# OxfordML/GPz

Hardware: AMD Instinct MI355X
Metric: objective+gradient evals/sec (higher is better)
Workload: dtype f64

## Files before the change

### gpz_amd/csrc/k_phi_quad.hip

```cpp
#include <float.h>
#include "gpz_dev.h"
#include "gpz_kernels.h"

template <int D>
struct PhiQuadShape {
    static constexpr int NT = D * (D + 1) / 2;
    static constexpr int NF = 1 + D + NT;
    static constexpr int NK = (NF + 3) / 4;
    static constexpr int CS = 4 * NK;
};

int phi_quad_stride(int de) { return 4 * ((1 + de + de * (de + 1) / 2 + 3) / 4); }
bool phi_quad_fits(int kind, int de, int mp, int k) { return kind == GPZ_KIND_COV && (de == 8 || de == 10) && mp > 256 && k == 1; }

template <int D>
__global__ __launch_bounds__(64) void k_phi_quad_coef(const double *__restrict__ Rc, const double *__restrict__ P,
                                                        const double *__restrict__ xmu, const double *__restrict__ fmx, int m, int mp,
                                                        double *__restrict__ Cq, double *__restrict__ blockmax,
                                                        unsigned *__restrict__ ticket, double *__restrict__ bound,
                                                        int *__restrict__ route) {
    constexpr int NT = PhiQuadShape<D>::NT, NF = PhiQuadShape<D>::NF, CS = PhiQuadShape<D>::CS, NP = NT + D;
    const int j = blockIdx.x * 64 + threadIdx.x;
    double bj = 0.0;
    if (j < m) {
        double R[NT], pq[D], u[D], uh[D];
        const double *rj = Rc + (size_t)j * NP;
#pragma unroll
        for (int e = 0; e < NT; ++e) R[e] = rj[e];
#pragma unroll
        for (int a = 0; a < D; ++a) pq[a] = P[(size_t)j * D + a] - xmu[a];
#pragma unroll
        for (int a = 0; a < D; ++a) {
            double s = 0.0, sh = 0.0;
#pragma unroll
            for (int b = a; b < D; ++b) {
                const double r = R[a * D - a * (a - 1) / 2 + (b - a)];
                s = fma(r, pq[b], s);
                sh = fma(fabs(r), fabs(pq[b]), sh);
            }
            u[a] = s; uh[a] = sh;
        }
        double *o = Cq + (size_t)j * CS;
        double c0 = 0.0, c0h = 0.0;
#pragma unroll
        for (int a = 0; a < D; ++a) { c0 = fma(u[a], u[a], c0); c0h = fma(uh[a], uh[a], c0h); }
        o[0] = -0.5 * c0;
        double bs = fmx[0] * (0.5 * c0h);
#pragma unroll
        for (int a = 0; a < D; ++a) {
            double s = 0.0, sh = 0.0;
#pragma unroll
            for (int r = 0; r <= a; ++r) {
                const double v = R[r * D - r * (r - 1) / 2 + (a - r)];
                s = fma(v, u[r], s);
                sh = fma(fabs(v), uh[r], sh);
            }
            o[1 + a] = s;
            bs = fma(fmx[1 + a], sh, bs);
        }
#pragma unroll
        for (int a = 0; a < D; ++a)
#pragma unroll
            for (int b = a; b < D; ++b) {
                double s = 0.0, sh = 0.0;
#pragma unroll
                for (int r = 0; r <= a; ++r) {
                    const double va = R[r * D - r * (r - 1) / 2 + (a - r)], vb = R[r * D - r * (r - 1) / 2 + (b - r)];
                    s = fma(va, vb, s);
                    sh = fma(fabs(va), fabs(vb), sh);
                }
                const int f = 1 + D + a * D - a * (a - 1) / 2 + (b - a);
                const double sc = (a == b) ? 0.5 : 1.0;
                o[f] = -sc * s;
                bs = fma(fmx[f], sc * sh, bs);
            }
#pragma unroll
        for (int f = NF; f < CS; ++f) o[f] = 0.0;
        bj = (double)(NF + 2 * D + 6) * 0x1p-53 * bs;
        if (!(bj <= DBL_MAX)) bj = __longlong_as_double(0x7ff0000000000000LL);
    } else if (j < mp) {
        double *o = Cq + (size_t)j * CS;
#pragma unroll
        for (int f = 0; f < CS; ++f) o[f] = 0.0;
    }
#pragma unroll
    for (int off = 32; off > 0; off >>= 1) bj = fmax(bj, __shfl_xor(bj, off, 64));
    int last = 0;
    if (threadIdx.x == 0) {
        blockmax[blockIdx.x] = bj;
        __threadfence();
        last = atomicAdd(ticket, 1u) == gridDim.x - 1 ? 1 : 0;
        if (last) {
            __threadfence();
            double mx = 0.0;
            for (unsigned g = 0; g < gridDim.x; ++g) mx = fmax(mx, __hip_atomic_load(blockmax + g, __ATOMIC_RELAXED, __HIP_MEMORY_SCOPE_AGENT));
            *bound = mx;
            *route = mx <= GPZ_PHI_QUAD_TAU ? GPZ_PHI_ROUTE_QUAD : GPZ_PHI_ROUTE_EXACT;
            *ticket = 0u;
        }
    }
}

int launch_phi_quad_coef(hipStream_t st, const double *Rc, const double *P, const double *xmu, const double *fmx, int m, int mp, int de,
                         double *Cq, double *blockmax, unsigned *ticket, double *bound, int *route) {
    dim3 g((mp + 63) / 64), b(64);
    switch (de) {
        case 8: hipLaunchKernelGGL(k_phi_quad_coef<8>, g, b, 0, st, Rc, P, xmu, fmx, m, mp, Cq, blockmax, ticket, bound, route); break;
        case 10: hipLaunchKernelGGL(k_phi_quad_coef<10>, g, b, 0, st, Rc, P, xmu, fmx, m, mp, Cq, blockmax, ticket, bound, route); break;
        default: return -1;
    }
    return 0;
}

struct PhiQuadKArgs {
    const double *Xs;
    const double *Cq;
    const int *route;
    int n, m, mp;
    const double *v, *bvec, *omega, *Y;
    double *Phi, *lnbeta, *wbeta;
    int jgroup;
    double *part;
    long ldp;
};

#ifndef GPZ_PHI_QUAD_RB
#define GPZ_PHI_QUAD_RB 2
#endif
#ifndef GPZ_PHI_QUAD_WGS
#define GPZ_PHI_QUAD_WGS 3
#endif

template <int D, int RB>
__global__ __launch_bounds__(256, GPZ_PHI_QUAD_WGS) void k_phi_quad(PhiQuadKArgs a) {
    constexpr int NF = PhiQuadShape<D>::NF, NK = PhiQuadShape<D>::NK, CS = PhiQuadShape<D>::CS, XL = D + 2;
    constexpr int NPB = 16 * CS;
    constexpr int NLD = (NPB + 255) / 256;
    if (*a.route != GPZ_PHI_ROUTE_QUAD) return;
    __shared__ double cq[2][NPB];
    __shared__ unsigned char pia[CS], pib[CS];
    const int tid = threadIdx.x, lane = tid & 63, wave = tid >> 6, li = lane & 15, lk = lane >> 4;
    const long row0 = ((long)blockIdx.x * 4 + wave) * (16 * RB);

    if (tid < CS) {
        const int f = tid;
        int ia = 0, ib = 0;
        if (f >= NF) ia = ib = XL - 1;
        else if (f >= 1) {
            if (f <= D) ia = f;
            else {
                int e2 = f - 1 - D, aa = 0;
                while (e2 >= D - aa) { e2 -= D - aa; ++aa; }
                ia = aa + 1; ib = aa + e2 + 1;
            }
        }
        pia[f] = (unsigned char)ia; pib[f] = (unsigned char)ib;
    }
    const int jlo = blockIdx.y * a.jgroup;
    const int jhi = min(a.mp, jlo + a.jgroup);
    double stg[NLD];
    auto pload = [&](int j0) {
#pragma unroll
        for (int q = 0; q < NLD; ++q) {
            const int e = tid + 256 * q;
            stg[q] = e < NPB ? a.Cq[(size_t)j0 * CS + e] : 0.0;
        }
    };
    auto pstore = [&](int buf) {
#pragma unroll
        for (int q = 0; q < NLD; ++q) {
            const int e = tid + 256 * q;
            if (e < NPB) cq[buf][e] = stg[q];
        }
    };
    pload(jlo);
    pstore(0);
    __syncthreads();

    double F[RB][NK];
#pragma unroll
    for (int ks = 0; ks < NK; ++ks) {
        const int ia = pia[4 * ks + lk], ib = pib[4 * ks + lk];
#pragma unroll
        for (int rb = 0; rb < RB; ++rb) {
            const long i = row0 + 16 * rb + li;
            const double *xr = a.Xs + (size_t)i * XL;
            F[rb][ks] = xr[ia] * xr[ib];
        }
    }
    double sv[RB][4];
#pragma unroll
    for (int rb = 0; rb < RB; ++rb)
#pragma unroll
        for (int r = 0; r < 4; ++r) sv[rb][r] = 0.0;

    int cur = 0;
    for (int j0 = jlo; j0 < jhi; j0 += 16, cur ^= 1) {
        const bool more = j0 + 16 < jhi;
        if (more) pload(j0 + 16);
        const int j = j0 + li;
        const double vj = (a.v && j < a.m) ? a.v[j] : 0.0;
        d4_t acc[RB];
#pragma unroll
        for (int rb = 0; rb < RB; ++rb) acc[rb] = d4_t{0.0, 0.0, 0.0, 0.0};
        const double *cb = &cq[cur][li * CS + lk];
#pragma unroll
        for (int ks = 0; ks < NK; ++ks) {
            const double b = cb[4 * ks];
#pragma unroll
            for (int rb = 0; rb < RB; ++rb) acc[rb] = MFMA_F64(F[rb][ks], b, acc[rb]);
        }
        double ph[RB][4];
#pragma unroll
        for (int rb = 0; rb < RB; ++rb) {
#pragma unroll
            for (int r = 0; r < 4; ++r) {
                const long i = row0 + 16 * rb + lk + 4 * r;
                const double e = exp(fmin(acc[rb][r], 0.0));
                ph[rb][r] = i < a.n ? e : 0.0;
                sv[rb][r] = fma(ph[rb][r], vj, sv[rb][r]);
            }
        }
        if (j0 + 16 > a.m) {
#pragma unroll
            for (int rb = 0; rb < RB; ++rb) {
#pragma unroll
                for (int r = 0; r < 4; ++r) {
                    const double y = a.Y ? a.Y[row0 + 16 * rb + lk + 4 * r] : 0.0;
                    if (j >= a.m) ph[rb][r] = j == a.m ? y : 0.0;
                }
            }
        }
        double *const po = a.Phi + (size_t)(row0 + lk) * a.mp + j;
#pragma unroll
        for (int rb = 0; rb < RB; ++rb) {
#pragma unroll
            for (int r = 0; r < 4; ++r) po[(size_t)(16 * rb + 4 * r) * a.mp] = ph[rb][r];
        }
        if (more) pstore(cur ^ 1);
        __syncthreads();
    }

#pragma unroll
    for (int rb = 0; rb < RB; ++rb)
#pragma unroll
        for (int r = 0; r < 4; ++r) {
#pragma unroll
            for (int off = 1; off < 16; off <<= 1) sv[rb][r] += __shfl_xor(sv[rb][r], off, 64);
        }
    if (li != 0) return;
#pragma unroll
    for (int rb = 0; rb < RB; ++rb)
#pragma unroll
        for (int r = 0; r < 4; ++r) {
            const long i = row0 + 16 * rb + lk + 4 * r;
            if (a.part) {
                if (i < a.ldp) {
                    a.part[((size_t)blockIdx.y * 2 + 0) * a.ldp + i] = sv[rb][r];
                    a.part[((size_t)blockIdx.y * 2 + 1) * a.ldp + i] = 0.0;
                }
                continue;
            }
            const bool valid = i < a.n;
            const double lb = a.bvec[0] + sv[rb][r];
            a.lnbeta[i] = valid ? lb : 0.0;
            if (a.wbeta) {
                const double om = a.omega ? a.omega[i] : 1.0;
                a.wbeta[i] = valid ? om * exp(-lb) : 0.0;
            }
        }
}

template <int D>
static int launch_phi_quad_d(hipStream_t st, const PhiArgs &a, const double *Xs, const double *Cq) {
    constexpr int RB = GPZ_PHI_QUAD_RB, JB = 16;
    const int rows_per_wg = 4 * 16 * RB;
    if (a.n_pad <= 0 || a.n_pad % rows_per_wg != 0 || a.n_pad > a.ldx) return -1;
    const int nwg = a.n_pad / rows_per_wg;
    int ngroup = 1;
    if (a.part && nwg < 1024) {
        int maxg = a.mp / (4 * JB);
        if (maxg > a.part_groups) maxg = a.part_groups;
        ngroup = phi_pick_groups(nwg, a.mp, JB, 2, 16, maxg < 1 ? 1 : maxg);
    }
    int jgroup = ((a.mp + ngroup - 1) / ngroup + JB - 1) / JB * JB;
    ngroup = (a.mp + jgroup - 1) / jgroup;
    PhiQuadKArgs q{};
    q.Xs = Xs; q.Cq = Cq; q.route = a.route; q.n = a.n; q.m = a.m; q.mp = a.mp;
    q.v = a.v; q.bvec = a.b; q.omega = a.omega; q.Y = a.Y;
    q.Phi = a.Phi; q.lnbeta = a.lnbeta; q.wbeta = a.wbeta;
    q.jgroup = jgroup; q.part = ngroup > 1 ? a.part : nullptr; q.ldp = (long)a.n_pad;
    hipLaunchKernelGGL((k_phi_quad<D, RB>), dim3(nwg, ngroup), dim3(256), 0, st, q);
    if (q.part)
        launch_phi_finalize(st, q.part, ngroup, a, a.route, GPZ_PHI_ROUTE_QUAD);
    return hipGetLastError() == hipSuccess ? 0 : -1;
}

int launch_phi_quad(hipStream_t st, const PhiArgs &a, const double *Xs, const double *Cq) {
    if (a.k != 1 || a.mp % 16 != 0 || !a.route || a.wgtab || !a.Phi || !a.lnbeta || a.w || a.phiw) return -1;
    switch (a.d) {
        case 8: return launch_phi_quad_d<8>(st, a, Xs, Cq);
        case 10: return launch_phi_quad_d<10>(st, a, Xs, Cq);
        default: return -1;
    }
}
```

### gpz_amd/csrc/k_gemm.hip

```cpp
#include <type_traits>
#include "gpz_dev.h"
#include "gpz_kernels.h"

#ifdef GPZ_GEMM_TRACE
__device__ unsigned long long *g_gemm_trace = nullptr;
#define GPZ_TRACE_MARK(slot)                                                                                              \
    do {                                                                                                                  \
        if (g_gemm_trace && (threadIdx.x & 63) == 0)                                                                      \
            g_gemm_trace[((size_t)item * 8 + (threadIdx.x >> 6)) * 6 + (slot)] = __builtin_amdgcn_s_memtime();       \
    } while (0)
#else
#define GPZ_TRACE_MARK(slot) do { } while (0)
#endif
typedef float f4_t __attribute__((ext_vector_type(4)));
typedef float f2_t __attribute__((ext_vector_type(2)));
#ifndef GPZ_F32_FLUSH
#define GPZ_F32_FLUSH 8
#endif
template <typename OT> struct MfmaOf;
template <> struct MfmaOf<double> {
    typedef d4_t acc_t;
    typedef d2_t pair_t;
    static __device__ __forceinline__ acc_t run(double a, double b, acc_t c) { return MFMA_F64(a, b, c); }
};
template <> struct MfmaOf<float> {
    typedef f4_t acc_t;
    typedef f2_t pair_t;
    static __device__ __forceinline__ acc_t run(float a, float b, acc_t c) { return __builtin_amdgcn_mfma_f32_16x16x4f32(a, b, c, 0, 0, 0); }
};
template <typename OT>
__device__ __forceinline__ typename MfmaOf<OT>::pair_t to_pair(const f2_t v) {
    typename MfmaOf<OT>::pair_t r;
    r.x = (OT)v.x;
    r.y = (OT)v.y;
    return r;
}
template <typename BT> struct Pair2 { typedef d2_t t; };
template <> struct Pair2<float> { typedef f2_t t; };
template <typename OT>
__device__ __forceinline__ typename MfmaOf<OT>::pair_t to_pair(const d2_t v) {
    typename MfmaOf<OT>::pair_t r;
    r.x = (OT)v.x;
    r.y = (OT)v.y;
    return r;
}

template <bool WEIGHTED, int WC, bool DIAGT, typename OT>
__device__ __forceinline__ void syrk_body(const double *__restrict__ Phi, int ld, const double *__restrict__ wgt,
                                          int mp, int i0, int j0, int r_begin, int r_end,
                                          double *__restrict__ out, OT (*sA)[16][LDS_LD128],
                                          OT (*sB)[16][LDS_LD128], OT (*sW)[16]) {
    constexpr int NT = 128 * WC;
    constexpr int NI = 8 / WC;
    constexpr int Q = 1024 / NT;
    constexpr bool diag_tile = DIAGT;
    constexpr bool PRESCALE = WEIGHTED;
    const int tid = threadIdx.x, lane = tid & 63, wave = tid >> 6;
    const int wr = wave / WC, wc = wave % WC;

    constexpr bool F32 = std::is_same<OT, float>::value;
    typedef typename MfmaOf<OT>::acc_t acc_t;
    typedef typename MfmaOf<OT>::pair_t pair_t;
    acc_t acc[4][NI];
    d4_t acc64[F32 ? 4 : 1][F32 ? NI : 1];
#pragma unroll
    for (int a = 0; a < 4; ++a)
#pragma unroll
        for (int b = 0; b < NI; ++b) {
            acc[a][b] = (acc_t){0, 0, 0, 0};
            if (F32) acc64[a][b] = (d4_t){0.0, 0.0, 0.0, 0.0};
        }
    auto flush = [&]() {
        if constexpr (F32) {
#pragma unroll
            for (int a = 0; a < 4; ++a)
#pragma unroll
                for (int b = 0; b < NI; ++b) {
#pragma unroll
                    for (int r = 0; r < 4; ++r) acc64[a][b][r] += (double)acc[a][b][r];
                    acc[a][b] = (acc_t){0, 0, 0, 0};
                }
        }
    };

    d2_t ra[Q], rb[Q];
    double rw = 0.0, rwq[PRESCALE ? Q : 1];
    const int ca = min(i0 + (tid & 63) * 2, mp - 2), cb = min(j0 + (tid & 63) * 2, mp - 2);
    const unsigned voa = (unsigned)(((tid >> 6) * ld + ca) * 8), vob = (unsigned)(((tid >> 6) * ld + cb) * 8);
    const unsigned vow = (unsigned)((PRESCALE ? (tid >> 6) : (tid & 15)) * 8);
    const size_t qsp = (size_t)(NT / 64) * ld * 8, ksp = (size_t)16 * ld * 8;
    const char *pp = reinterpret_cast<const char *>(Phi + (size_t)r_begin * ld);
    const char *pw = reinterpret_cast<const char *>(WEIGHTED ? wgt + r_begin : nullptr);
    auto gload = [&]() {
        unsigned oa = voa, ob = vob, ow = vow;
        asm volatile("" : "+v"(oa), "+v"(ob), "+v"(ow));
#pragma unroll
        for (int q = 0; q < Q; ++q) {
            ra[q] = *reinterpret_cast<const d2_t *>(pp + q * qsp + oa);
            if (!diag_tile) rb[q] = *reinterpret_cast<const d2_t *>(pp + q * qsp + ob);
            if (PRESCALE) rwq[q] = *reinterpret_cast<const double *>(pw + q * (NT / 64) * 8 + ow);
        }
        if (WEIGHTED && !PRESCALE && tid < 16) rw = *reinterpret_cast<const double *>(pw + ow);
        pp += ksp;
        if (WEIGHTED) pw += 16 * 8;
    };
    auto lstore = [&](int buf) {
#pragma unroll
        for (int q = 0; q < Q; ++q) {
            int idx = q * NT + tid;
            int row = idx >> 6, c = (idx & 63) * 2;
            if (diag_tile) *reinterpret_cast<pair_t *>(&sB[buf][row][c]) = to_pair<OT>(ra[q]);
            else *reinterpret_cast<pair_t *>(&sB[buf][row][c]) = to_pair<OT>(rb[q]);
            if (PRESCALE) { ra[q].x *= rwq[q]; ra[q].y *= rwq[q]; }
            *reinterpret_cast<pair_t *>(&sA[buf][row][c]) = to_pair<OT>(ra[q]);
        }
        if (WEIGHTED && !PRESCALE && tid < 16) sW[buf][tid] = (OT)rw;
    };

    const int nstage = (r_end > r_begin) ? (r_end - r_begin) / 16 : 0;
    if (nstage > 0) {
        gload();
        lstore(0);
        if (nstage > 1) gload();
    }
    __syncthreads();
    static_assert(!DIAGT || NI == 2, "diagonal-tile wave roles are written for the 2 x 4 wave grid");
    constexpr int NA = 4, NB = DIAGT ? 5 : NI;
    int dra[5] = {0, 0, 0, 0, 0}, dcb[5] = {0, 0, 0, 0, 0};
    bool has5 = false;
    if (DIAGT) {
        const int wv = __builtin_amdgcn_readfirstlane(wave);
        const unsigned RA[8] = {0x00000u, 0x11111u, 0x22222u, 0x33333u, 0x77000u, 0x66611u, 0x55552u, 0x44444u};
        const unsigned CB[8] = {0x43210u, 0x54321u, 0x65432u, 0x76543u, 0x77765u, 0x77676u, 0x77657u, 0x77654u};
        has5 = wv < 4;
#pragma unroll
        for (int p = 0; p < 5; ++p) {
            dra[p] = (RA[wv] >> (4 * p)) & 15;
            dcb[p] = (CB[wv] >> (4 * p)) & 15;
        }
    }
    auto rdfrag = [&](int cur, int kk, OT (&a)[NA], OT (&b)[NB]) {
        const OT(*tA)[LDS_LD128] = sA[cur];
        const OT(*tB)[LDS_LD128] = sB[cur];
        const int krow = kk * 4 + (lane >> 4);
        if (DIAGT) {
#pragma unroll
            for (int p = 0; p < 4; ++p) a[p] = tA[krow][dra[p] * 16 + (lane & 15)];
#pragma unroll
            for (int p = 0; p < 5; ++p) b[p] = tB[krow][dcb[p] * 16 + (lane & 15)];
        } else {
#pragma unroll
            for (int mi = 0; mi < 4; ++mi) a[mi] = tA[krow][wr * 64 + mi * 16 + (lane & 15)];
#pragma unroll
            for (int ni = 0; ni < NI; ++ni) b[ni] = tB[krow][wc * (16 * NI) + ni * 16 + (lane & 15)];
        }
    };
    auto burst = [&](const OT (&a)[NA], const OT (&b)[NB]) {
        __builtin_amdgcn_s_setprio(1);
        if (DIAGT) {
#pragma unroll
            for (int p = 0; p < 4; ++p) acc[p][0] = MfmaOf<OT>::run(a[p], b[p], acc[p][0]);
            if (has5) acc[0][1] = MfmaOf<OT>::run(a[0], b[DIAGT ? 4 : 0], acc[0][1]);
        } else {
#pragma unroll
            for (int mi = 0; mi < 4; ++mi)
#pragma unroll
                for (int ni = 0; ni < NI; ++ni) acc[mi][ni] = MfmaOf<OT>::run(a[mi], b[ni], acc[mi][ni]);
        }
        __builtin_amdgcn_s_setprio(0);
    };
    OT fa0[NA] = {}, fb0[NB] = {}, fa1[NA] = {}, fb1[NB] = {};
    if (nstage > 0) rdfrag(0, 0, fa0, fb0);
    auto stage = [&](auto curc, int s) {
        constexpr int cur = decltype(curc)::value;
        rdfrag(cur, 1, fa1, fb1);
        __builtin_amdgcn_sched_barrier(0);
        burst(fa0, fb0);
        __builtin_amdgcn_sched_barrier(0);
        rdfrag(cur, 2, fa0, fb0);
        __builtin_amdgcn_sched_barrier(0);
        burst(fa1, fb1);
        __builtin_amdgcn_sched_barrier(0);
        if (s + 1 < nstage) {
            lstore(cur ^ 1);
            if (s + 2 < nstage) gload();
        }
        rdfrag(cur, 3, fa1, fb1);
        __builtin_amdgcn_sched_barrier(0);
        burst(fa0, fb0);
        __builtin_amdgcn_sched_barrier(0);
        __syncthreads();
        if (s + 1 < nstage) rdfrag(cur ^ 1, 0, fa0, fb0);
        __builtin_amdgcn_sched_barrier(0);
        burst(fa1, fb1);
        __builtin_amdgcn_sched_barrier(0);
    };
    int s = 0;
    for (; s + 1 < nstage; s += 2) {
        stage(std::integral_constant<int, 0>{}, s);
        stage(std::integral_constant<int, 1>{}, s + 1);
        if (F32 && ((s + 2) % GPZ_F32_FLUSH) == 0) flush();
    }
    if (s < nstage) stage(std::integral_constant<int, 0>{}, s);
    flush();
    auto res = [&](int mi, int ni, int r) -> double {
        if constexpr (F32) return acc64[mi][ni][r];
        else return acc[mi][ni][r];
    };
    auto crow = [&](int r) -> int { return F32 ? 4 * (lane >> 4) + r : (lane >> 4) + 4 * r; };

    if (DIAGT) {
#pragma unroll
        for (int p = 0; p < 5; ++p) {
            if (p == 4 && !has5) break;
            const int col = j0 + dcb[p] * 16 + (lane & 15);
#pragma unroll
            for (int r = 0; r < 4; ++r) {
                const int row = i0 + dra[p] * 16 + crow(r);
                if (row < mp && col < mp) out[(size_t)row * mp + col] = p < 4 ? res(p, 0, r) : res(0, 1, r);
            }
        }
    } else {
#pragma unroll
        for (int mi = 0; mi < 4; ++mi)
#pragma unroll
            for (int ni = 0; ni < NI; ++ni) {
                const int col = j0 + wc * (16 * NI) + ni * 16 + (lane & 15);
#pragma unroll
                for (int r = 0; r < 4; ++r) {
                    const int row = i0 + wr * 64 + mi * 16 + crow(r);
                    if (row < mp && col < mp) out[(size_t)row * mp + col] = res(mi, ni, r);
                }
            }
    }
}

template <bool WEIGHTED, bool TRI, int WC, typename OT>
__global__ __launch_bounds__(128 * WC, (std::is_same<OT, float>::value ? 2 : WC)) void k_syrk(
    const double *__restrict__ Phi, int ld, const double *__restrict__ wgt, int n_rows, int mp, int ntile, int nsplit,
    int rows_per_split, int nsplit_d, int rows_per_split_d, double *__restrict__ slab) {
    __shared__ OT sA[2][16][LDS_LD128];
    __shared__ OT sB[2][16][LDS_LD128];
    __shared__ OT sW[2][16];

    const int npairs = ntile * (ntile + 1) / 2;
    const int nwg = gridDim.x, xcd = blockIdx.x & 7, qq = nwg >> 3, rr = nwg & 7;
    const int lb = (xcd < rr ? xcd * (qq + 1) : rr * (qq + 1) + (xcd - rr) * qq) + (blockIdx.x >> 3);
    const int noff = npairs - ntile, ndiag = ntile * nsplit_d;
    auto gstart = [&](int g) { return g * noff + g * ndiag / nsplit; };
    int g = (int)((unsigned)lb * (unsigned)nsplit / (unsigned)(noff * nsplit + ndiag));
    g = g > nsplit - 1 ? nsplit - 1 : g;
    while (g > 0 && gstart(g) > lb) --g;
    while (g + 1 < nsplit && gstart(g + 1) <= lb) ++g;
    const int within = lb - gstart(g);
    int ti, tj, split, rps;
    if (within < noff) {
        split = g;
        rps = rows_per_split;
        int rem = within;
        ti = 0;
        while (rem >= ntile - 1 - ti) { rem -= ntile - 1 - ti; ++ti; }
        tj = ti + 1 + rem;
    } else {
        const int q = g * ndiag / nsplit + within - noff;
        split = q / ntile;
        rps = rows_per_split_d;
        ti = tj = q % ntile;
    }
    const bool diag_tile = (ti == tj);
    const int i0 = ti * 128, j0 = tj * 128;

    int r_begin = split * rps;
    int r_end = min(n_rows, r_begin + rps);
    if (TRI) r_begin = max(r_begin, j0 & ~15);
    double *out = slab + (size_t)split * mp * mp;
    if (diag_tile)
        syrk_body<WEIGHTED, WC, true, OT>(Phi, ld, wgt, mp, i0, j0, r_begin, r_end, out, sA, sB, sW);
    else
        syrk_body<WEIGHTED, WC, false, OT>(Phi, ld, wgt, mp, i0, j0, r_begin, r_end, out, sA, sB, sW);
}

__global__ void k_syrk_reduce(const double *__restrict__ slab, int nsplit_off, int nsplit_d, int mp,
                              double *__restrict__ S, int lds, int accumulate) {
    const int j = blockIdx.x * blockDim.x + threadIdx.x;
    const int i = blockIdx.y;
    if (j >= mp || i > j) return;
    const int ti = i >> 7, tj = j >> 7;
    const int nsplit = (ti == tj) ? nsplit_d : nsplit_off;
    const size_t stride = (size_t)mp * mp;
    const double *p = slab + (size_t)i * mp + j;
    double s0 = 0.0, s1 = 0.0, s2 = 0.0, s3 = 0.0;
    int k = 0;
    for (; k + 8 <= nsplit; k += 8) {
        double v[8];
#pragma unroll
        for (int q = 0; q < 8; ++q) v[q] = p[(size_t)(k + q) * stride];
        s0 += v[0]; s1 += v[1]; s2 += v[2]; s3 += v[3];
        s0 += v[4]; s1 += v[5]; s2 += v[6]; s3 += v[7];
    }
    for (; k < nsplit; ++k) s0 += p[(size_t)k * stride];
    const double t = (s0 + s1) + (s2 + s3);
    S[(size_t)i * lds + j] = accumulate ? S[(size_t)i * lds + j] + t : t;
    if (i != j) S[(size_t)j * lds + i] = accumulate ? S[(size_t)j * lds + i] + t : t;
}

template <bool EDGE, int WC, typename OT, typename BT>
__device__ __forceinline__ void tgemm_body(const double *__restrict__ Phi, int ld, const BT *__restrict__ B,
                                           int ldb, double *__restrict__ T, int ldt, int mp, int i0, int j0,
                                           OT (*sA)[128][18], OT (*sB)[16][LDS_LD128],
                                           double *__restrict__ nupart, double *__restrict__ phiw, int m, int mcol,
                                           long n_pad, int ct, int kdim, int ncol16 = 8, int slot = 0, int nslot = 1, int item = 0) {
    constexpr int NT = 128 * WC;
    constexpr int NI = 8 / WC;
    constexpr int Q = 1024 / NT;
    const int tid = threadIdx.x, lane = tid & 63, wave = tid >> 6;
    const int wr = wave / WC, wc = wave % WC;

    typedef typename MfmaOf<OT>::acc_t acc_t;
    typedef typename MfmaOf<OT>::pair_t pair_t;
    acc_t acc[4][NI];
#pragma unroll
    for (int a = 0; a < 4; ++a)
#pragma unroll
        for (int b = 0; b < NI; ++b) acc[a][b] = (acc_t){0, 0, 0, 0};

    typedef typename Pair2<BT>::t bpair_t;
    d2_t ra[Q];
    bpair_t rb[Q];
    const unsigned voa = (unsigned)(((tid >> 3) * ld + (tid & 7) * 2) * 8);
    const unsigned vob = (unsigned)(((tid >> 6) * ldb + min(j0 + (tid & 63) * 2, mp - 2)) * sizeof(BT));
    const size_t qsa = (size_t)(NT / 8) * ld * 8, qsb = (size_t)(NT / 64) * ldb * sizeof(BT), ksb = (size_t)16 * ldb * sizeof(BT);
    const char *pa = reinterpret_cast<const char *>(Phi + (size_t)i0 * ld);
    const char *pb = reinterpret_cast<const char *>(B);
    auto gload = [&]() {
        unsigned oa = voa, ob = vob;
        asm volatile("" : "+v"(oa), "+v"(ob));
#pragma unroll
        for (int q = 0; q < Q; ++q) {
            ra[q] = *reinterpret_cast<const d2_t *>(pa + q * qsa + oa);
            rb[q] = *reinterpret_cast<const bpair_t *>(pb + q * qsb + ob);
        }
        pa += 16 * 8;
        pb += ksb;
    };
    auto lstore = [&](int buf) {
#pragma unroll
        for (int q = 0; q < Q; ++q) {
            int idx = q * NT + tid;
            int arow = idx >> 3, ac = (idx & 7) * 2;
            *reinterpret_cast<pair_t *>(&sA[buf][arow][ac]) = to_pair<OT>(ra[q]);
            int row = idx >> 6, c = (idx & 63) * 2;
            *reinterpret_cast<pair_t *>(&sB[buf][row][c]) = to_pair<OT>(rb[q]);
        }
    };

    int nvalid = NI;
    if (EDGE) {
        nvalid = (mp - j0 + 15) / 16;
        nvalid = nvalid < 0 ? 0 : (nvalid > ncol16 ? ncol16 : nvalid);
        nvalid = __builtin_amdgcn_readfirstlane(nvalid);
    }
    static_assert(!EDGE || 4 * NI == 8, "the row-strip deal keeps its eight accumulators in acc[4][2]");
    constexpr int NFA = EDGE ? 1 : 4, NFB = EDGE ? 8 : NI;

    const int nstage = kdim / 16;
    gload();
    lstore(0);
    if (nstage > 1) gload();
    __syncthreads();
    auto rdfrag = [&](int cur, int kk, OT (&a)[NFA], OT (&b)[NFB]) {
        const int kc = kk * 4 + (lane >> 4);
        if (EDGE) {
            a[0] = sA[cur][wave * 16 + (lane & 15)][kc];
#pragma unroll
            for (int p = 0; p < NFB; ++p) b[p] = sB[cur][kc][p * 16 + (lane & 15)];
        } else {
#pragma unroll
            for (int mi = 0; mi < NFA; ++mi) a[mi] = sA[cur][wr * 64 + mi * 16 + (lane & 15)][kc];
#pragma unroll
            for (int ni = 0; ni < NI; ++ni) b[ni] = sB[cur][kc][wc * (16 * NI) + ni * 16 + (lane & 15)];
        }
    };
    auto burst = [&](const OT (&a)[NFA], const OT (&b)[NFB]) {
        __builtin_amdgcn_s_setprio(1);
        if (EDGE) {
#pragma unroll
            for (int p = 0; p < NFB; ++p)
                if (p < nvalid) acc[p >> 1][p & 1] = MfmaOf<OT>::run(a[0], b[p], acc[p >> 1][p & 1]);
        } else {
#pragma unroll
            for (int ni = 0; ni < NI; ++ni) {
#pragma unroll
                for (int mi = 0; mi < NFA; ++mi) acc[mi][ni] = MfmaOf<OT>::run(a[mi], b[ni], acc[mi][ni]);
            }
        }
        __builtin_amdgcn_s_setprio(0);
    };
    OT fa0[NFA], fb0[NFB], fa1[NFA], fb1[NFB];
    rdfrag(0, 0, fa0, fb0);
    GPZ_TRACE_MARK(1);
    auto stage = [&](auto curc, int s) {
        constexpr int cur = decltype(curc)::value;
        rdfrag(cur, 1, fa1, fb1);
        __builtin_amdgcn_sched_barrier(0);
        burst(fa0, fb0);
        __builtin_amdgcn_sched_barrier(0);
        rdfrag(cur, 2, fa0, fb0);
        __builtin_amdgcn_sched_barrier(0);
        burst(fa1, fb1);
        __builtin_amdgcn_sched_barrier(0);
        if (s + 1 < nstage) {
            lstore(cur ^ 1);
            if (s + 2 < nstage) gload();
        }
        rdfrag(cur, 3, fa1, fb1);
        __builtin_amdgcn_sched_barrier(0);
        burst(fa0, fb0);
        __builtin_amdgcn_sched_barrier(0);
        __syncthreads();
        if (s + 1 < nstage) rdfrag(cur ^ 1, 0, fa0, fb0);
        __builtin_amdgcn_sched_barrier(0);
        burst(fa1, fb1);
        __builtin_amdgcn_sched_barrier(0);
    };
    int s = 0;
    for (; s + 1 < nstage; s += 2) {
        stage(std::integral_constant<int, 0>{}, s);
        stage(std::integral_constant<int, 1>{}, s + 1);
    }
    if (s < nstage) stage(std::integral_constant<int, 0>{}, s);
    GPZ_TRACE_MARK(2);
    auto res = [&](int mi, int ni, int r) -> double { return (double)acc[mi][ni][r]; };
    auto crow = [&](int r) -> int { return std::is_same<OT, float>::value ? 4 * (lane >> 4) + r : (lane >> 4) + 4 * r; };

    if (EDGE) {
#pragma unroll
        for (int p = 0; p < NFB; ++p) {
            const int col = j0 + p * 16 + (lane & 15);
            if (p < nvalid && col < mp) {
#pragma unroll
                for (int r = 0; r < 4; ++r) T[(size_t)(i0 + wave * 16 + crow(r)) * ldt + col] = res(p >> 1, p & 1, r);
            }
        }
        if (nupart) {
#pragma unroll
            for (int r = 0; r < 4; ++r) {
                const int row = i0 + wave * 16 + crow(r);
                double pp = 0.0;
#pragma unroll
                for (int p = 0; p < NFB; ++p) {
                    const int col = j0 + p * 16 + (lane & 15);
                    if (p < nvalid && col < m) pp = fma(Phi[(size_t)row * ld + col], res(p >> 1, p & 1, r), pp);
                    if (p < nvalid && col == mcol) phiw[row] = res(p >> 1, p & 1, r);
                }
                pp += __shfl_xor(pp, 1, 64);
                pp += __shfl_xor(pp, 2, 64);
                pp += __shfl_xor(pp, 4, 64);
                pp += __shfl_xor(pp, 8, 64);
                if ((lane & 15) == 0) {
                    nupart[(size_t)(ct * WC + slot) * n_pad + row] = pp;
                    if (slot == 0)
#pragma unroll
                        for (int q = 1; q < WC; ++q)
                            if (q >= nslot) nupart[(size_t)(ct * WC + q) * n_pad + row] = 0.0;
                }
            }
        }
        return;
    }
    const int wv = __builtin_amdgcn_readfirstlane(wave);
    const int wru = wv / WC, wcu = wv % WC;
    const char *pbase = reinterpret_cast<const char *>(Phi + (size_t)(i0 + wru * 64) * ld + j0 + wcu * (16 * NI));
    char *tbase = reinterpret_cast<char *>(T + (size_t)(i0 + wru * 64) * ldt + j0 + wcu * (16 * NI));
    double *slotp = nupart ? nupart + (size_t)(ct * WC + wc) * n_pad : nullptr;
#pragma unroll
    for (int hf = 0; hf < 2; ++hf) {
        double ph[2][4][NI];
        if (nupart) {
#pragma unroll
            for (int mh = 0; mh < 2; ++mh)
#pragma unroll
                for (int r = 0; r < 4; ++r)
#pragma unroll
                    for (int ni = 0; ni < NI; ++ni)
                        ph[mh][r][ni] = *reinterpret_cast<const double *>(pbase + ((size_t)((hf * 2 + mh) * 16 + crow(r)) * ld + ni * 16 + (lane & 15)) * 8);
        }
        __builtin_amdgcn_sched_barrier(0);
#pragma unroll
        for (int mh = 0; mh < 2; ++mh)
#pragma unroll
            for (int ni = 0; ni < NI; ++ni) {
#pragma unroll
                for (int r = 0; r < 4; ++r)
                    *reinterpret_cast<double *>(tbase + ((size_t)((hf * 2 + mh) * 16 + crow(r)) * ldt + ni * 16 + (lane & 15)) * 8) = res(hf * 2 + mh, ni, r);
            }
        __builtin_amdgcn_sched_barrier(0);
        if (nupart) {
#pragma unroll
            for (int mh = 0; mh < 2; ++mh)
#pragma unroll
                for (int r = 0; r < 4; ++r) {
                    const int mi = hf * 2 + mh;
                    const int row = i0 + wr * 64 + mi * 16 + crow(r);
                    double p = 0.0;
#pragma unroll
                    for (int ni = 0; ni < NI; ++ni) {
                        const int col = j0 + wc * (16 * NI) + ni * 16 + (lane & 15);
                        const double t = fma(ph[mh][r][ni], res(mi, ni, r), p);
                        p = (col < m) ? t : p;
                        if (col == mcol) phiw[row] = res(mi, ni, r);
                    }
                    p += __shfl_xor(p, 1, 64);
                    p += __shfl_xor(p, 2, 64);
                    p += __shfl_xor(p, 4, 64);
                    p += __shfl_xor(p, 8, 64);
                    if ((lane & 15) == 0) slotp[row] = p;
                }
        }
        __builtin_amdgcn_sched_barrier(0);
    }
}

template <int WC, typename OT, typename BT>
__global__ __launch_bounds__(128 * WC, WC) void k_tgemm(const double *__restrict__ Phi, int ld,
                                                        const BT *__restrict__ B, int ldb,
                                                        double *__restrict__ T, int ldt, int mp, int nct,
                                                        double *__restrict__ nupart, double *__restrict__ phiw, int m,
                                                        int mcol, long n_pad, int kdim, int nfull, int npiece) {
    __shared__ OT sA[2][128][18];
    __shared__ OT sB[2][16][LDS_LD128];
    const int item = blockIdx.x;
#ifdef GPZ_GEMM_TRACE
    GPZ_TRACE_MARK(0);
    if (g_gemm_trace && (threadIdx.x & 63) == 0)
        g_gemm_trace[((size_t)item * 8 + (threadIdx.x >> 6)) * 6 + 4] =
            ((unsigned long long)__builtin_amdgcn_s_getreg((31 << 11) | 20) << 32) | __builtin_amdgcn_s_getreg((31 << 11) | 4);
    struct TraceEnd { int item; __device__ ~TraceEnd() { GPZ_TRACE_MARK(3); } } trace_end{item};
#endif
    if (item >= nfull) {
        const int q = item - nfull;
        const int tile = nfull + q / npiece, piece = q % npiece;
        const int rt = tile / nct, ct = tile % nct;
        tgemm_body<true, WC, OT, BT>(Phi, ld, B, ldb, T, ldt, mp, rt * 128, ct * 128 + piece * (128 / npiece), sA, sB, nupart, phiw, m, mcol,
                                 n_pad, ct, kdim, 8 / npiece, piece, npiece, item);
        return;
    }
    const int nwg = nfull, xcd = item & 7, q = nwg >> 3, r = nwg & 7;
    const int lb = (xcd < r ? xcd * (q + 1) : r * (q + 1) + (xcd - r) * q) + (item >> 3);
    const int rt = lb / nct, ct = lb % nct;
    const int i0 = rt * 128, j0 = ct * 128;
    if (j0 + 128 <= mp)
        tgemm_body<false, WC, OT, BT>(Phi, ld, B, ldb, T, ldt, mp, i0, j0, sA, sB, nupart, phiw, m, mcol, n_pad, ct, kdim, 8, 0, 1, item);
    else
        tgemm_body<true, WC, OT, BT>(Phi, ld, B, ldb, T, ldt, mp, i0, j0, sA, sB, nupart, phiw, m, mcol, n_pad, ct, kdim, 8, 0, 1, item);
}

__device__ void gemm_tile_64(const double *__restrict__ A, long lda, const double *__restrict__ B, long ldb,
                             double *__restrict__ C, long ldc, int M, int N, int kbeg, int kend, double alpha, int tm,
                             int tn) {
    __shared__ double sA[2][16][LDS_LD64];
    __shared__ double sB[2][16][LDS_LD64];
    const int tid = threadIdx.x, lane = tid & 63, wave = tid >> 6;
    const int wr = wave >> 1, wc = wave & 1;
    const int i0 = tm * 64, j0 = tn * 64;
    d4_t acc[2][2];
#pragma unroll
    for (int a = 0; a < 2; ++a)
#pragma unroll
        for (int b = 0; b < 2; ++b) acc[a][b] = (d4_t){0.0, 0.0, 0.0, 0.0};

    const int ar = tid >> 2, ak = (tid & 3) * 4;
    const int bk = tid >> 4, bc = (tid & 15) * 4;
    const bool aok = i0 + ar < M, bok = j0 + bc < N;
    const double *ap = A + (size_t)(i0 + ar) * lda + ak;
    const double *bp = B + (size_t)bk * ldb + j0 + bc;
    struct Regs { d2_t a[2], b[2]; } r0, r1;
    auto gload = [&](Regs &r, int k0) {
        const d2_t z = {0.0, 0.0};
        r.a[0] = aok ? *reinterpret_cast<const d2_t *>(ap + k0) : z;
        r.a[1] = aok ? *reinterpret_cast<const d2_t *>(ap + k0 + 2) : z;
        r.b[0] = bok ? *reinterpret_cast<const d2_t *>(bp + (size_t)k0 * ldb) : z;
        r.b[1] = bok ? *reinterpret_cast<const d2_t *>(bp + (size_t)k0 * ldb + 2) : z;
    };
// ... 147 lines not shown
```

Baseline: 18.94.

## Use exp2 with log2e-folded coefficients and specialize Phi loop for full tiles

Folds log2(e) into the quadratic coefficients so the Phi kernel can evaluate a custom polynomial exp2 on non-positive inputs instead of the library exp, and widens the error bound to cover the extra rounding. The basis loop is templated on a row-guard flag so full row tiles skip per-element n checks. Phi stores now go through a scalar base pointer plus a fixed per-lane offset, and the wave index is made uniform with readfirstlane, to cut VGPR address arithmetic. Tail columns at or beyond m are written in a separate pass after the main store. The risk is slightly different rounding in exp, plus larger code from the duplicated loop.

```diff
diff --git a/gpz_amd/csrc/k_exp.h b/gpz_amd/csrc/k_exp.h
--- /dev/null
+++ b/gpz_amd/csrc/k_exp.h
@@ -0,0 +1,48 @@
+#pragma once
+#include <math.h>
+
+#if defined(__HIPCC__) || defined(__CUDACC__)
+#define GPZ_EXP_HD __host__ __device__
+#else
+#define GPZ_EXP_HD
+#endif
+
+GPZ_EXP_HD inline double gpz_exp2_poly(double r) {
+    double q = 0x1.e9d3fe3952179p-32;
+    q = fma(q, r, 0x1.e6063f7217bc6p-28);
+    q = fma(q, r, 0x1.b524fae627834p-24);
+    q = fma(q, r, 0x1.62bfd47773353p-20);
+    q = fma(q, r, 0x1.ffcbfc670dcd4p-17);
+    q = fma(q, r, 0x1.430913096fd9fp-13);
+    q = fma(q, r, 0x1.5d87fe78a5276p-10);
+    q = fma(q, r, 0x1.3b2ab6fba1ddap-7);
+    q = fma(q, r, 0x1.c6b08d704a0c2p-5);
+    q = fma(q, r, 0x1.ebfbdff82c598p-3);
+    q = fma(q, r, 0x1.62e42fefa39efp-1);
+    return fma(r, q, 1.0);
+}
+
+GPZ_EXP_HD inline double gpz_exp2_nonpos(double t) {
+    t = fmax(fmin(t, 0.0), -1080.0);
+    const double k = rint(t);
+    return ldexp(gpz_exp2_poly(t - k), (int)k);
+}
+
+GPZ_EXP_HD inline double gpz_exp_nonpos(double x) {
+    x = fmax(fmin(x, 0.0), -750.0);
+    const double k = rint(x * 0x1.71547652b82fep+0);
+    double s = fma(-k, 0x1.62e42fee00000p-1, x);
+    s = fma(-k, 0x1.a39ef35793c76p-33, s);
+    double q = 0x1.af4de6a36d4fcp-26;
+    q = fma(q, s, 0x1.28a2c810d05b6p-22);
+    q = fma(q, s, 0x1.71de0232f4775p-19);
+    q = fma(q, s, 0x1.a019a6635643cp-16);
+    q = fma(q, s, 0x1.a01a01abe78f9p-13);
+    q = fma(q, s, 0x1.6c16c17f45e48p-10);
+    q = fma(q, s, 0x1.11111111100dcp-7);
+    q = fma(q, s, 0x1.55555555520a7p-5);
+    q = fma(q, s, 0x1.5555555555557p-3);
+    q = fma(q, s, 0x1.0000000000005p-1);
+    q = fma(q, s, 1.0);
+    return ldexp(fma(s, q, 1.0), (int)k);
+}
diff --git a/gpz_amd/csrc/k_phi_quad.hip b/gpz_amd/csrc/k_phi_quad.hip
--- a/gpz_amd/csrc/k_phi_quad.hip
+++ b/gpz_amd/csrc/k_phi_quad.hip
@@ -1,6 +1,21 @@
 #include <float.h>
+#include <type_traits>
 #include "gpz_dev.h"
 #include "gpz_kernels.h"
+#include "k_exp.h"
+
+#ifndef GPZ_PHI_QUAD_EXP2
+#define GPZ_PHI_QUAD_EXP2 1
+#endif
+#ifndef GPZ_PHI_QUAD_FASTROWS
+#define GPZ_PHI_QUAD_FASTROWS 1
+#endif
+#ifndef GPZ_PHI_QUAD_SADDR
+#define GPZ_PHI_QUAD_SADDR 1
+#endif
+#ifndef GPZ_PHI_QUAD_NT
+#define GPZ_PHI_QUAD_NT 0
+#endif
 
 template <int D>
 struct PhiQuadShape {
@@ -41,10 +56,15 @@
             u[a] = s; uh[a] = sh;
         }
         double *o = Cq + (size_t)j * CS;
+#if GPZ_PHI_QUAD_EXP2
+        constexpr double L2E = 0x1.71547652b82fep+0;
+#else
+        constexpr double L2E = 1.0;
+#endif
         double c0 = 0.0, c0h = 0.0;
 #pragma unroll
         for (int a = 0; a < D; ++a) { c0 = fma(u[a], u[a], c0); c0h = fma(uh[a], uh[a], c0h); }
-        o[0] = -0.5 * c0;
+        o[0] = L2E * (-0.5 * c0);
         double bs = fmx[0] * (0.5 * c0h);
 #pragma unroll
         for (int a = 0; a < D; ++a) {
@@ -55,7 +75,7 @@
                 s = fma(v, u[r], s);
                 sh = fma(fabs(v), uh[r], sh);
             }
-            o[1 + a] = s;
+            o[1 + a] = L2E * s;
             bs = fma(fmx[1 + a], sh, bs);
         }
 #pragma unroll
@@ -71,12 +91,12 @@
                 }
                 const int f = 1 + D + a * D - a * (a - 1) / 2 + (b - a);
                 const double sc = (a == b) ? 0.5 : 1.0;
-                o[f] = -sc * s;
+                o[f] = L2E * (-sc * s);
                 bs = fma(fmx[f], sc * sh, bs);
             }
 #pragma unroll
         for (int f = NF; f < CS; ++f) o[f] = 0.0;
-        bj = (double)(NF + 2 * D + 6) * 0x1p-53 * bs;
+        bj = (double)(NF + 2 * D + 6 + (GPZ_PHI_QUAD_EXP2 ? 2 : 0)) * 0x1p-53 * bs;
         if (!(bj <= DBL_MAX)) bj = __longlong_as_double(0x7ff0000000000000LL);
     } else if (j < mp) {
         double *o = Cq + (size_t)j * CS;
@@ -139,7 +159,8 @@
     if (*a.route != GPZ_PHI_ROUTE_QUAD) return;
     __shared__ double cq[2][NPB];
     __shared__ unsigned char pia[CS], pib[CS];
-    const int tid = threadIdx.x, lane = tid & 63, wave = tid >> 6, li = lane & 15, lk = lane >> 4;
+    const int tid = threadIdx.x, lane = tid & 63, li = lane & 15, lk = lane >> 4;
+    const int wave = __builtin_amdgcn_readfirstlane(tid >> 6);
     const long row0 = ((long)blockIdx.x * 4 + wave) * (16 * RB);
 
     if (tid < CS) {
@@ -194,52 +215,85 @@
 #pragma unroll
         for (int r = 0; r < 4; ++r) sv[rb][r] = 0.0;
 
-    int cur = 0;
-    for (int j0 = jlo; j0 < jhi; j0 += 16, cur ^= 1) {
-        const bool more = j0 + 16 < jhi;
-        if (more) pload(j0 + 16);
-        const int j = j0 + li;
-        const double vj = (a.v && j < a.m) ? a.v[j] : 0.0;
-        d4_t acc[RB];
-#pragma unroll
-        for (int rb = 0; rb < RB; ++rb) acc[rb] = d4_t{0.0, 0.0, 0.0, 0.0};
-        const double *cb = &cq[cur][li * CS + lk];
-#pragma unroll
-        for (int ks = 0; ks < NK; ++ks) {
-            const double b = cb[4 * ks];
-#pragma unroll
-            for (int rb = 0; rb < RB; ++rb) acc[rb] = MFMA_F64(F[rb][ks], b, acc[rb]);
-        }
-        double ph[RB][4];
-#pragma unroll
-        for (int rb = 0; rb < RB; ++rb) {
-#pragma unroll
-            for (int r = 0; r < 4; ++r) {
-                const long i = row0 + 16 * rb + lk + 4 * r;
-                const double e = exp(fmin(acc[rb][r], 0.0));
-                ph[rb][r] = i < a.n ? e : 0.0;
-                sv[rb][r] = fma(ph[rb][r], vj, sv[rb][r]);
-            }
-        }
-        if (j0 + 16 > a.m) {
+    char *pw = reinterpret_cast<char *>(a.Phi + (size_t)row0 * a.mp + jlo);
+    const unsigned vo = (unsigned)((lk * a.mp + li) * 8);
+    auto phi_store = [](double *p, double x) {
+#if GPZ_PHI_QUAD_NT
+        __builtin_nontemporal_store(x, p);
+#else
+        *p = x;
+#endif
+    };
+
+    auto basis_loop = [&](auto guardc) {
+        constexpr bool GUARD = decltype(guardc)::value;
+        int cur = 0;
+        for (int j0 = jlo; j0 < jhi; j0 += 16, cur ^= 1) {
+            const bool more = j0 + 16 < jhi;
+            if (more) pload(j0 + 16);
+            const int j = j0 + li;
+            const double vj = (a.v && j < a.m) ? a.v[j] : 0.0;
+            d4_t acc[RB];
+#pragma unroll
+            for (int rb = 0; rb < RB; ++rb) acc[rb] = d4_t{0.0, 0.0, 0.0, 0.0};
+            const double *cb = &cq[cur][li * CS + lk];
+#pragma unroll
+            for (int ks = 0; ks < NK; ++ks) {
+                const double b = cb[4 * ks];
+#pragma unroll
+                for (int rb = 0; rb < RB; ++rb) acc[rb] = MFMA_F64(F[rb][ks], b, acc[rb]);
+            }
+            double ph[RB][4];
 #pragma unroll
             for (int rb = 0; rb < RB; ++rb) {
 #pragma unroll
                 for (int r = 0; r < 4; ++r) {
-                    const double y = a.Y ? a.Y[row0 + 16 * rb + lk + 4 * r] : 0.0;
-                    if (j >= a.m) ph[rb][r] = j == a.m ? y : 0.0;
+#if GPZ_PHI_QUAD_EXP2
+                    const double e = gpz_exp2_nonpos(fmin(acc[rb][r], 0.0));
+#else
+                    const double e = exp(fmin(acc[rb][r], 0.0));
+#endif
+                    ph[rb][r] = !GUARD || row0 + 16 * rb + lk + 4 * r < a.n ? e : 0.0;
+                    sv[rb][r] = fma(ph[rb][r], vj, sv[rb][r]);
                 }
             }
-        }
-        double *const po = a.Phi + (size_t)(row0 + lk) * a.mp + j;
-#pragma unroll
-        for (int rb = 0; rb < RB; ++rb) {
-#pragma unroll
-            for (int r = 0; r < 4; ++r) po[(size_t)(16 * rb + 4 * r) * a.mp] = ph[rb][r];
-        }
-        if (more) pstore(cur ^ 1);
-        __syncthreads();
-    }
+#if GPZ_PHI_QUAD_SADDR
+            unsigned o = vo;
+            asm volatile("" : "+v"(o));
+#pragma unroll
+            for (int rb = 0; rb < RB; ++rb) {
+#pragma unroll
+                for (int r = 0; r < 4; ++r) phi_store(reinterpret_cast<double *>(pw + (size_t)(16 * rb + 4 * r) * a.mp * 8 + o), ph[rb][r]);
+            }
+            pw += 16 * 8;
+#else
+            double *const po = a.Phi + (size_t)(row0 + lk) * a.mp + j;
+#pragma unroll
+            for (int rb = 0; rb < RB; ++rb) {
+#pragma unroll
+                for (int r = 0; r < 4; ++r) phi_store(po + (size_t)(16 * rb + 4 * r) * a.mp, ph[rb][r]);
+            }
+#endif
+            if (j0 + 16 > a.m && j >= a.m) {
+#pragma unroll
+                for (int rb = 0; rb < RB; ++rb) {
+#pragma unroll
+                    for (int r = 0; r < 4; ++r) {
+                        const long i = row0 + 16 * rb + lk + 4 * r;
+                        a.Phi[(size_t)i * a.mp + j] = (j == a.m && a.Y) ? a.Y[i] : 0.0;
+                    }
+                }
+            }
+            if (more) pstore(cur ^ 1);
+            __syncthreads();
+        }
+    };
+#if GPZ_PHI_QUAD_FASTROWS
+    if (row0 + 16 * RB <= a.n) basis_loop(std::false_type{});
+    else basis_loop(std::true_type{});
+#else
+    basis_loop(std::true_type{});
+#endif
 
 #pragma unroll
     for (int rb = 0; rb < RB; ++rb)
```

Measured after the change: 18.96, median of 4. About the same (+0.1%).

## Use buffer loads and inline-asm LDS reads with explicit lgkmcnt waits in GEMM kernels

Applied to the files above, without the earlier changes.

Replaces the global loads in the syrk and GEMM stage loaders with raw buffer loads that carry per-slice resource descriptors and scalar offsets. Replaces the compiler-generated LDS fragment reads with inline ds_read instructions that use compile-time immediate offsets from precomputed base addresses. Explicit lgkmcnt waits let the next fragment's reads stay in flight while the current MFMA burst runs. The aim is fewer address-computation VALU ops and conservative waits, at the cost of manual hazard management that could break if the compiler's own counter accounting interacts with the asm.

```diff
diff --git a/gpz_amd/csrc/k_gemm.hip b/gpz_amd/csrc/k_gemm.hip
--- a/gpz_amd/csrc/k_gemm.hip
+++ b/gpz_amd/csrc/k_gemm.hip
@@ -35,6 +35,34 @@
     r.y = (OT)v.y;
     return r;
 }
+template <int V> using ic_t = std::integral_constant<int, V>;
+template <typename OT> __device__ __forceinline__ unsigned lds_addr(const OT *p) {
+    return (unsigned)(size_t)(const __attribute__((address_space(3))) void *)p;
+}
+template <int OFF, typename OT> __device__ __forceinline__ void lds_get(OT &v, unsigned base) {
+    static_assert(OFF >= 0 && OFF < 65536, "LDS immediate offset");
+    if constexpr (sizeof(OT) == 8) asm volatile("ds_read_b64 %0, %1 offset:%2" : "=v"(v) : "v"(base), "n"(OFF) : "memory");
+    else asm volatile("ds_read_b32 %0, %1 offset:%2" : "=v"(v) : "v"(base), "n"(OFF) : "memory");
+}
+template <int N, typename OT, int NA, int NB> __device__ __forceinline__ void lds_wait(OT (&a)[NA], OT (&b)[NB]) {
+    asm volatile("s_waitcnt lgkmcnt(%0)" ::"n"(N) : "memory");
+#pragma unroll
+    for (int i = 0; i < NA; ++i) asm volatile("" : "+v"(a[i]));
+#pragma unroll
+    for (int i = 0; i < NB; ++i) asm volatile("" : "+v"(b[i]));
+}
+__device__ __forceinline__ __amdgpu_buffer_rsrc_t slice_rsrc(const char *p) {
+    return __builtin_amdgcn_make_buffer_rsrc(const_cast<char *>(p), 0, -1, 0x00020000);
+}
+__device__ __forceinline__ d2_t bload16(__amdgpu_buffer_rsrc_t r, unsigned voff, int soff) {
+    return __builtin_bit_cast(d2_t, __builtin_amdgcn_raw_buffer_load_b128(r, (int)voff, soff, 0));
+}
+__device__ __forceinline__ f2_t bload8f(__amdgpu_buffer_rsrc_t r, unsigned voff, int soff) {
+    return __builtin_bit_cast(f2_t, __builtin_amdgcn_raw_buffer_load_b64(r, (int)voff, soff, 0));
+}
+__device__ __forceinline__ double bload8(__amdgpu_buffer_rsrc_t r, unsigned voff, int soff) {
+    return __builtin_bit_cast(double, __builtin_amdgcn_raw_buffer_load_b64(r, (int)voff, soff, 0));
+}
 template <typename BT> struct Pair2 { typedef d2_t t; };
 template <> struct Pair2<float> { typedef f2_t t; };
 template <typename OT>
@@ -92,15 +120,14 @@
     const char *pp = reinterpret_cast<const char *>(Phi + (size_t)r_begin * ld);
     const char *pw = reinterpret_cast<const char *>(WEIGHTED ? wgt + r_begin : nullptr);
     auto gload = [&]() {
-        unsigned oa = voa, ob = vob, ow = vow;
-        asm volatile("" : "+v"(oa), "+v"(ob), "+v"(ow));
+        const __amdgpu_buffer_rsrc_t rp = slice_rsrc(pp), rq = slice_rsrc(pw);
 #pragma unroll
         for (int q = 0; q < Q; ++q) {
-            ra[q] = *reinterpret_cast<const d2_t *>(pp + q * qsp + oa);
-            if (!diag_tile) rb[q] = *reinterpret_cast<const d2_t *>(pp + q * qsp + ob);
-            if (PRESCALE) rwq[q] = *reinterpret_cast<const double *>(pw + q * (NT / 64) * 8 + ow);
-        }
-        if (WEIGHTED && !PRESCALE && tid < 16) rw = *reinterpret_cast<const double *>(pw + ow);
+            ra[q] = bload16(rp, voa, q * (int)qsp);
+            if (!diag_tile) rb[q] = bload16(rp, vob, q * (int)qsp);
+            if (PRESCALE) rwq[q] = bload8(rq, vow, q * (NT / 64) * 8);
+        }
+        if (WEIGHTED && !PRESCALE && tid < 16) rw = *reinterpret_cast<const double *>(pw + vow);
         pp += ksp;
         if (WEIGHTED) pw += 16 * 8;
     };
@@ -139,20 +166,29 @@
             dcb[p] = (CB[wv] >> (4 * p)) & 15;
         }
     }
-    auto rdfrag = [&](int cur, int kk, OT (&a)[NA], OT (&b)[NB]) {
-        const OT(*tA)[LDS_LD128] = sA[cur];
-        const OT(*tB)[LDS_LD128] = sB[cur];
-        const int krow = kk * 4 + (lane >> 4);
-        if (DIAGT) {
-#pragma unroll
-            for (int p = 0; p < 4; ++p) a[p] = tA[krow][dra[p] * 16 + (lane & 15)];
-#pragma unroll
-            for (int p = 0; p < 5; ++p) b[p] = tB[krow][dcb[p] * 16 + (lane & 15)];
+    constexpr int SZ = (int)sizeof(OT), KOFF = 4 * LDS_LD128 * SZ, BUFOFF = 16 * LDS_LD128 * SZ, NRD = NA + NB;
+    unsigned fba[DIAGT ? 4 : 1], fbb[DIAGT ? 5 : 1];
+    if (DIAGT) {
+#pragma unroll
+        for (int p = 0; p < 4; ++p) fba[p] = lds_addr(&sA[0][lane >> 4][dra[p] * 16 + (lane & 15)]);
+#pragma unroll
+        for (int p = 0; p < 5; ++p) fbb[DIAGT ? p : 0] = lds_addr(&sB[0][lane >> 4][dcb[p] * 16 + (lane & 15)]);
+    } else {
+        fba[0] = lds_addr(&sA[0][lane >> 4][wr * 64 + (lane & 15)]);
+        fbb[0] = lds_addr(&sB[0][lane >> 4][wc * (16 * NI) + (lane & 15)]);
+    }
+    auto rdfrag = [&](auto curc, auto kkc, OT (&a)[NA], OT (&b)[NB]) {
+        constexpr int off = decltype(curc)::value * BUFOFF + decltype(kkc)::value * KOFF;
+        if constexpr (DIAGT) {
+            lds_get<off>(a[0], fba[0]); lds_get<off>(a[1], fba[1]); lds_get<off>(a[2], fba[2]); lds_get<off>(a[3], fba[3]);
+            lds_get<off>(b[0], fbb[0]); lds_get<off>(b[1], fbb[1]); lds_get<off>(b[2], fbb[2]); lds_get<off>(b[3], fbb[3]);
+            lds_get<off>(b[4], fbb[4]);
         } else {
-#pragma unroll
-            for (int mi = 0; mi < 4; ++mi) a[mi] = tA[krow][wr * 64 + mi * 16 + (lane & 15)];
-#pragma unroll
-            for (int ni = 0; ni < NI; ++ni) b[ni] = tB[krow][wc * (16 * NI) + ni * 16 + (lane & 15)];
+            lds_get<off>(a[0], fba[0]); lds_get<off + 16 * SZ>(a[1], fba[0]);
+            lds_get<off + 32 * SZ>(a[2], fba[0]); lds_get<off + 48 * SZ>(a[3], fba[0]);
+            lds_get<off>(b[0], fbb[0]);
+            if constexpr (NI > 1) lds_get<off + 16 * SZ>(b[1], fbb[0]);
+            if constexpr (NI > 2) { lds_get<off + 32 * SZ>(b[2], fbb[0]); lds_get<off + 48 * SZ>(b[3], fbb[0]); }
         }
     };
     auto burst = [&](const OT (&a)[NA], const OT (&b)[NB]) {
@@ -170,14 +206,16 @@
         __builtin_amdgcn_s_setprio(0);
     };
     OT fa0[NA] = {}, fb0[NB] = {}, fa1[NA] = {}, fb1[NB] = {};
-    if (nstage > 0) rdfrag(0, 0, fa0, fb0);
+    if (nstage > 0) rdfrag(ic_t<0>{}, ic_t<0>{}, fa0, fb0);
     auto stage = [&](auto curc, int s) {
         constexpr int cur = decltype(curc)::value;
-        rdfrag(cur, 1, fa1, fb1);
+        rdfrag(ic_t<cur>{}, ic_t<1>{}, fa1, fb1);
+        lds_wait<NRD>(fa0, fb0);
         __builtin_amdgcn_sched_barrier(0);
         burst(fa0, fb0);
         __builtin_amdgcn_sched_barrier(0);
-        rdfrag(cur, 2, fa0, fb0);
+        rdfrag(ic_t<cur>{}, ic_t<2>{}, fa0, fb0);
+        lds_wait<NRD>(fa1, fb1);
         __builtin_amdgcn_sched_barrier(0);
         burst(fa1, fb1);
         __builtin_amdgcn_sched_barrier(0);
@@ -185,23 +223,27 @@
             lstore(cur ^ 1);
             if (s + 2 < nstage) gload();
         }
-        rdfrag(cur, 3, fa1, fb1);
+        rdfrag(ic_t<cur>{}, ic_t<3>{}, fa1, fb1);
+        lds_wait<NRD>(fa0, fb0);
         __builtin_amdgcn_sched_barrier(0);
         burst(fa0, fb0);
         __builtin_amdgcn_sched_barrier(0);
+        lds_wait<0>(fa1, fb1);
         __syncthreads();
-        if (s + 1 < nstage) rdfrag(cur ^ 1, 0, fa0, fb0);
+        int nx = s + 1;
+        asm volatile("" : "+s"(nx));
+        if (nx < nstage) rdfrag(ic_t<(cur ^ 1)>{}, ic_t<0>{}, fa0, fb0);
         __builtin_amdgcn_sched_barrier(0);
         burst(fa1, fb1);
         __builtin_amdgcn_sched_barrier(0);
     };
     int s = 0;
     for (; s + 1 < nstage; s += 2) {
-        stage(std::integral_constant<int, 0>{}, s);
-        stage(std::integral_constant<int, 1>{}, s + 1);
+        stage(ic_t<0>{}, s);
+        stage(ic_t<1>{}, s + 1);
         if (F32 && ((s + 2) % GPZ_F32_FLUSH) == 0) flush();
     }
-    if (s < nstage) stage(std::integral_constant<int, 0>{}, s);
+    if (s < nstage) stage(ic_t<0>{}, s);
     flush();
     auto res = [&](int mi, int ni, int r) -> double {
         if constexpr (F32) return acc64[mi][ni][r];
@@ -333,12 +375,12 @@
     const char *pa = reinterpret_cast<const char *>(Phi + (size_t)i0 * ld);
     const char *pb = reinterpret_cast<const char *>(B);
     auto gload = [&]() {
-        unsigned oa = voa, ob = vob;
-        asm volatile("" : "+v"(oa), "+v"(ob));
+        const __amdgpu_buffer_rsrc_t rpa = slice_rsrc(pa), rpb = slice_rsrc(pb);
 #pragma unroll
         for (int q = 0; q < Q; ++q) {
-            ra[q] = *reinterpret_cast<const d2_t *>(pa + q * qsa + oa);
-            rb[q] = *reinterpret_cast<const bpair_t *>(pb + q * qsb + ob);
+            ra[q] = bload16(rpa, voa, q * (int)qsa);
+            if constexpr (std::is_same<BT, float>::value) rb[q] = bload8f(rpb, vob, q * (int)qsb);
+            else rb[q] = bload16(rpb, vob, q * (int)qsb);
         }
         pa += 16 * 8;
         pb += ksb;
@@ -368,17 +410,20 @@
     lstore(0);
     if (nstage > 1) gload();
     __syncthreads();
-    auto rdfrag = [&](int cur, int kk, OT (&a)[NFA], OT (&b)[NFB]) {
-        const int kc = kk * 4 + (lane >> 4);
-        if (EDGE) {
-            a[0] = sA[cur][wave * 16 + (lane & 15)][kc];
-#pragma unroll
-            for (int p = 0; p < NFB; ++p) b[p] = sB[cur][kc][p * 16 + (lane & 15)];
-        } else {
-#pragma unroll
-            for (int mi = 0; mi < NFA; ++mi) a[mi] = sA[cur][wr * 64 + mi * 16 + (lane & 15)][kc];
-#pragma unroll
-            for (int ni = 0; ni < NI; ++ni) b[ni] = sB[cur][kc][wc * (16 * NI) + ni * 16 + (lane & 15)];
+    constexpr int SZ = (int)sizeof(OT), NRD = NFA + NFB;
+    constexpr int ABUF = 128 * 18 * SZ, AK = 4 * SZ, AM = 16 * 18 * SZ, BBUF = 16 * LDS_LD128 * SZ, BK = 4 * LDS_LD128 * SZ, BN = 16 * SZ;
+    const unsigned fba = lds_addr(&sA[0][(EDGE ? wave * 16 : wr * 64) + (lane & 15)][lane >> 4]);
+    const unsigned fbb = lds_addr(&sB[0][lane >> 4][(EDGE ? 0 : wc * (16 * NI)) + (lane & 15)]);
+    auto rdfrag = [&](auto curc, auto kkc, OT (&a)[NFA], OT (&b)[NFB]) {
+        constexpr int oa = decltype(curc)::value * ABUF + decltype(kkc)::value * AK;
+        constexpr int ob = decltype(curc)::value * BBUF + decltype(kkc)::value * BK;
+        lds_get<oa>(a[0], fba);
+        if constexpr (!EDGE) { lds_get<oa + AM>(a[1], fba); lds_get<oa + 2 * AM>(a[2], fba); lds_get<oa + 3 * AM>(a[3], fba); }
+        lds_get<ob>(b[0], fbb);
+        if constexpr (NFB > 1) lds_get<ob + BN>(b[1], fbb);
+        if constexpr (NFB > 2) { lds_get<ob + 2 * BN>(b[2], fbb); lds_get<ob + 3 * BN>(b[3], fbb); }
+        if constexpr (NFB > 4) {
+            lds_get<ob + 4 * BN>(b[4], fbb); lds_get<ob + 5 * BN>(b[5], fbb); lds_get<ob + 6 * BN>(b[6], fbb); lds_get<ob + 7 * BN>(b[7], fbb);
         }
     };
     auto burst = [&](const OT (&a)[NFA], const OT (&b)[NFB]) {
@@ -397,15 +442,17 @@
         __builtin_amdgcn_s_setprio(0);
     };
     OT fa0[NFA], fb0[NFB], fa1[NFA], fb1[NFB];
-    rdfrag(0, 0, fa0, fb0);
+    rdfrag(ic_t<0>{}, ic_t<0>{}, fa0, fb0);
     GPZ_TRACE_MARK(1);
     auto stage = [&](auto curc, int s) {
         constexpr int cur = decltype(curc)::value;
-        rdfrag(cur, 1, fa1, fb1);
+        rdfrag(ic_t<cur>{}, ic_t<1>{}, fa1, fb1);
+        lds_wait<NRD>(fa0, fb0);
         __builtin_amdgcn_sched_barrier(0);
         burst(fa0, fb0);
         __builtin_amdgcn_sched_barrier(0);
-        rdfrag(cur, 2, fa0, fb0);
+        rdfrag(ic_t<cur>{}, ic_t<2>{}, fa0, fb0);
+        lds_wait<NRD>(fa1, fb1);
         __builtin_amdgcn_sched_barrier(0);
         burst(fa1, fb1);
         __builtin_amdgcn_sched_barrier(0);
@@ -413,22 +460,26 @@
             lstore(cur ^ 1);
             if (s + 2 < nstage) gload();
         }
-        rdfrag(cur, 3, fa1, fb1);
+        rdfrag(ic_t<cur>{}, ic_t<3>{}, fa1, fb1);
+        lds_wait<NRD>(fa0, fb0);
         __builtin_amdgcn_sched_barrier(0);
         burst(fa0, fb0);
         __builtin_amdgcn_sched_barrier(0);
+        lds_wait<0>(fa1, fb1);
         __syncthreads();
-        if (s + 1 < nstage) rdfrag(cur ^ 1, 0, fa0, fb0);
+        int nx = s + 1;
+        asm volatile("" : "+s"(nx));
+        if (nx < nstage) rdfrag(ic_t<(cur ^ 1)>{}, ic_t<0>{}, fa0, fb0);
         __builtin_amdgcn_sched_barrier(0);
         burst(fa1, fb1);
         __builtin_amdgcn_sched_barrier(0);
     };
     int s = 0;
     for (; s + 1 < nstage; s += 2) {
-        stage(std::integral_constant<int, 0>{}, s);
-        stage(std::integral_constant<int, 1>{}, s + 1);
-    }
-    if (s < nstage) stage(std::integral_constant<int, 0>{}, s);
+        stage(ic_t<0>{}, s);
+        stage(ic_t<1>{}, s + 1);
+    }
+    if (s < nstage) stage(ic_t<0>{}, s);
     GPZ_TRACE_MARK(2);
     auto res = [&](int mi, int ni, int r) -> double { return (double)acc[mi][ni][r]; };
     auto crow = [&](int r) -> int { return std::is_same<OT, float>::value ? 4 * (lane >> 4) + r : (lane >> 4) + 4 * r; };
```

Measured after the change: 19.03 before, 19.15 after (median of 6 runs). Within noise of the previous version (+0.6%).
